# lym01803/FinalProject-LosslessImageCompression

Measured on AMD Instinct MI355X. Metric: encode+decode Mpixels/s (imagenet64, bit-exact round trip), higher is better.
Workload: dtype f32

## Files before the change

finalproject-losslessimagecompression_amd/csrc/conv3_dx3.hip:

```cpp
#include <hip/hip_runtime.h>
#include <stdint.h>

#include <utility>

#include "idf_cdf.h"
#include "idf_codec_internal.h"
#include "wino_common.h"

#pragma clang fp contract(off)

namespace idf {

typedef float d4 __attribute__((ext_vector_type(4)));
typedef _Float16 e4 __attribute__((ext_vector_type(4)));
typedef _Float16 e8 __attribute__((ext_vector_type(8)));
typedef unsigned int v4u __attribute__((ext_vector_type(4)));
typedef __bf16 b8 __attribute__((ext_vector_type(8)));

struct Dx3Args {
  const uint16_t* xs;
  int64_t P;
  int64_t xs_pix, xs_slab, xs_bytes;
  int32_t nslab_xs;
  int32_t C;
  const uint16_t* Wt;
  int32_t nslab, ngroup;
  int32_t N;
  int32_t B, H, Wd;
  int32_t nbx, nby;
  int32_t tiles_x, tiles_y, ntiles, nblk_tiles;
  int32_t ch;
  int32_t seg, segw, nseg;
  int32_t gut, wp, hp;
  int32_t tilew, xskip;
  int32_t nchunk, chunk_slabs;
  float* part;
  uint32_t* ctr;
  const float* b3;
  const float* vtap;
  const float* bfull;
  int32_t ldv;
  int32_t act;
  float slope;
  float* out;
  int64_t ldo;
  float yscale;
  uint32_t* flag;
  const float* hw;
  int32_t ldhw, nh;
  float* hacc;
  int32_t hlast, skip_f32, hmode, hn_mean;
  float* hout;
  int64_t hld_out;
  const float* hbase;
  int64_t hld_base;
  float *hmean, *hlogs, *hscale;
};

#ifndef IDF_DX3_ABLATE
#define IDF_DX3_ABLATE 0
#endif
#ifndef IDF_DX3_DB
#define IDF_DX3_DB 3
#endif
#ifndef IDF_DX3_SB
#define IDF_DX3_SB 1
#endif
// ... 7 lines not shown
#define IDF_DX3_STAG 0
#endif
#ifndef IDF_DX3_STAMPS
#define IDF_DX3_STAMPS 0
#endif
#ifndef IDF_DX3_STAMP_BLOCK
#define IDF_DX3_STAMP_BLOCK 100
#endif
#if IDF_DX3_STAMPS
__device__ unsigned long long g_dx3_stamp[8][40][4];
__device__ unsigned long long g_dx3_phase[8][6];
#define DX3_PHASE(j, v)                                                                      \
  do {                                                                                      \
    if (blockIdx.x == IDF_DX3_STAMP_BLOCK && lane == 0) g_dx3_phase[wave][(j)] = (v);       \
  } while (0)
#define DX3_STAMP(slab, j)                                                                 \
  do {                                                                                    \
    if (blockIdx.x == IDF_DX3_STAMP_BLOCK && (slab) < 40 && lane == 0)                    \
      g_dx3_stamp[wave][(slab)][(j)] = __builtin_amdgcn_s_memtime();                      \
  } while (0)
#else
#define DX3_STAMP(slab, j) do { } while (0)
#define DX3_PHASE(j, v) do { } while (0)
#endif
#ifndef IDF_DX3_TL
#define IDF_DX3_TL 0
#endif
#if IDF_DX3_TL
__device__ unsigned long long g_dx3_tl[4096][8];
#define DX3_TL(j)                                                                          \
  do {                                                                                    \
    if (tid == 0 && blockIdx.x < 4096) g_dx3_tl[blockIdx.x][(j)] = __builtin_amdgcn_s_memrealtime(); \
  } while (0)
#else
#define DX3_TL(j) do { } while (0)
#endif
#ifndef IDF_DX3_KSPLIT
#define IDF_DX3_KSPLIT 4
#endif
#ifndef IDF_DX3_KSPLIT16
#define IDF_DX3_KSPLIT16 1
#endif
#ifndef IDF_DX3_TWO_MIN
#define IDF_DX3_TWO_MIN 512
#endif
#ifndef IDF_DX3_FORCE1
#define IDF_DX3_FORCE1 0
#endif

#ifndef IDF_DX3_PAIRS
#define IDF_DX3_PAIRS 0
#endif
#ifndef IDF_DX3_PRIO
#define IDF_DX3_PRIO 0
#endif
#ifndef IDF_DX3_PRIO_K
#define IDF_DX3_PRIO_K 4
#endif
#ifndef IDF_DX3_MIX
#define IDF_DX3_MIX 0
#endif
#ifndef IDF_DX3_WAVES
#define IDF_DX3_WAVES 8
#endif
constexpr int kDxWaves = IDF_DX3_WAVES;
constexpr int kDxThreads = 64 * kDxWaves;
constexpr uint32_t kDxInvalid = 0xFFFFFFF0u;
constexpr uint32_t kDxOff = 0x80000000u;
// ... 137 lines not shown
  static_assert(HR >= 3, "the A-fragment reads of a phase take its last three steps");
  static_assert(IDF_DX3_DMAS == 0 || IDF_DX3_DMA0 + IDF_DX3_STAG + (L::PPW - 1) * IDF_DX3_DMAS < NS,
                "every DMA piece of a slab is issued within the slab's steps");
  int* last_flag = (int*)(lds + L::FOFF);
  const int tid = threadIdx.x, lane = tid & 63;
  const int wave = __builtin_amdgcn_readfirstlane(tid >> 6);
  const int bid = xcd_contiguous(blockIdx.x, gridDim.x);
  const int per_chunk = g.ngroup * g.nblk_tiles;
  const int chunk = udiv_s(bid, per_chunk);
  const int rem = bid - chunk * per_chunk;
  const int grp = udiv_s(rem, g.nblk_tiles);
  const int tb = rem - grp * g.nblk_tiles;
  const int tw = MIX ? (wave & 3) >> 1 : wave / (kDxWaves / T);
  constexpr int WR_OLD = IDF_DX3_MIX == 2 ? WR - 1 : WR + 1;
  const int r0 = MIX ? 2 * WR * (wave & 1) + ((wave & 4) ? WR_OLD : 0) : WR * (wave % (kDxWaves / T));
  d4 hreg[WRW];
  const int nlayers = ML ? ml->nlayers : 1;
  for (int li = 0; li < nlayers; ++li) {
  int tid_o = tid, lane_o = lane, wave_o = wave, tb_o = tb, tw_o = tw, r0_o = r0, grp_o = grp,
      chunk_o = chunk;
  if constexpr (ML) {
    asm volatile("" : "+v"(tid_o), "+v"(lane_o), "+v"(wave_o), "+v"(tb_o), "+v"(tw_o), "+v"(r0_o),
                 "+v"(grp_o), "+v"(chunk_o));
    wave_o = __builtin_amdgcn_readfirstlane(wave_o);
    tb_o = __builtin_amdgcn_readfirstlane(tb_o);
    tw_o = __builtin_amdgcn_readfirstlane(tw_o);
    r0_o = __builtin_amdgcn_readfirstlane(r0_o);
    grp_o = __builtin_amdgcn_readfirstlane(grp_o);
    chunk_o = __builtin_amdgcn_readfirstlane(chunk_o);
  }
  const int tid = tid_o, lane = lane_o, wave = wave_o, tb = tb_o, tw = tw_o, r0 = r0_o,
            grp = grp_o, chunk = chunk_o;
  const int lz = 0;
  Dx3Layer Ly;
  if constexpr (ML) {
    Ly = ml->layer[li];
  } else {
    Ly = Dx3Layer{g.Wt, g.b3, g.vtap, g.bfull, g.out, g.yscale, g.C, g.nslab, g.nchunk,
                  g.chunk_slabs, g.hlast};
  }
  const int tile = tb * T + tw + lz;

  const int64_t plane_b = g.P * 32;
  const int xs_rec = (int)(g.xs_slab < (int64_t)kDxInvalid ? g.xs_slab : (int64_t)kDxInvalid);
  uint32_t pbase[L::PPW];
  int plo[L::PPW];
  bool pok[L::PPW];
#pragma unroll
  for (int i = 0; i < L::PPW; ++i) {
    const bool hk = i < L::PH;
    const int k = wave + kDxWaves * (hk ? i : i - L::PH);
    pok[i] = k < (hk ? L::HPIECES : L::WPIECES);
    pbase[i] = kDxOff;
    plo[i] = 0;
    if (hk && pok[i]) {
      const int t = k / (L::NPL * PLANE_KIB), pl = (k / PLANE_KIB) % L::NPL, pi = k % PLANE_KIB;
      plo[i] = (t * L::NPL + pl) * L::PLANE + pi * 1024;
      const int slot = 32 * pi + (lane >> 1);
      const int tt = tb * T + t;
      if (tt < g.ntiles) {
        const DxTile dt = dx_tile(g, tt);
        int ix, x, iy, y;
        bool ok;
        if (g.gut) {
          const int cr = slot / PITCH, cc = slot - cr * PITCH;
          const int u = dt.u0 - 1 + cc, uy = dt.u0y - 1 + cr;
          ix = u >= 0 ? udiv_s(u, g.wp) : 0;
          x = u >= 0 ? u - ix * g.wp : -1;
          iy = uy >= 0 ? udiv_s(uy, g.hp) : 0;
          y = uy >= 0 ? uy - iy * g.hp : -1;
          ok = cr < g.ch && cc < g.segw;
        } else {
          const int sk = g.seg ? udiv_s(slot, g.seg) : 0;
          const int rr = slot - sk * g.seg;
          const int cr = rr / PITCH, cc = rr - cr * PITCH;
          ok = sk < g.nseg && cc < g.segw && cr < g.ch;
          ix = dt.ix0 + sk;
          x = (sk ? 0 : dt.xf0) - 1 + cc;
          const int vy = dt.vy0 + cr;
          iy = udiv_s(vy, g.H + 2);
          y = vy - iy * (g.H + 2) - 1;
        }
        const int b = (dt.band * g.nby + iy) * g.nbx + ix;
        ok = ok && x >= 0 && x < g.Wd && ix < g.nbx && y >= 0 && y < g.H && iy < g.nby && b < g.B;
        if (ok)
          pbase[i] = (uint32_t)(pl * plane_b + ((((int64_t)b * g.H + y) * g.Wd + x) * g.xs_pix) + (lane & 1) * 16);
      }
    } else if (!hk && pok[i]) {
      plo[i] = L::WOFF + k * 1024;
      pbase[i] = (uint32_t)(grp * L::WST + k * 1024 + lane * 16);
    }
  }
  DX3_TL(0);
  for (int e = tid; e < NF * 512 / 16; e += kDxThreads) *(d4*)(lds + L::ZOFF + 16 * e) = d4{0.f, 0.f, 0.f, 0.f};
  DX3_PHASE(0, __builtin_amdgcn_s_memtime());
  DX3_PHASE(4, __builtin_amdgcn_s_memrealtime());

  const int j = lane & 15, q = lane >> 4;
  const DxTile dt = dx_tile(g, tile < g.ntiles ? tile : 0);
  const int jx = g.xskip ? 3 * (j >> 1) + (j & 1) : j;
  const int uj = dt.u0 + jx;
  const int pw = g.gut ? g.wp : g.Wd;
  const int ixj = udiv_s(uj, pw);
  const int xj = uj - ixj * pw;
  const int kj = ixj - dt.ix0;
  const int colb = g.gut ? jx : kj * g.seg + (kj ? j - (ixj * g.Wd - dt.u0) : j);
  const int uyw = dt.u0y + r0;
  int iyw = udiv_s(uyw, g.H);
  if (iyw > g.nby - 1) iyw = g.nby - 1;
  const int rowb = g.gut ? r0 : uyw + 2 * iyw - dt.vy0;

  const int slot0 = rowb * PITCH + colb;
  const int tb0 = tw * L::NPL * L::PLANE;
  const int oP = tb0 + (q >> 1) * L::PLANE + slot0 * 32 + (q & 1) * 16;
  const int oF = tb0 + slot0 * 32 + (q & 1) * 16 + (q >> 1) * 32;
  const int oG = tb0 + slot0 * 32 + (q & 1) * 16 + 64 + (q >> 1) * PITCH * 32;
  const int oAH = L::WOFF + j * 32 + (q & 1) * 16;
  constexpr int WLO = BF ? 0 : L::WPART;
  const int oAF = L::WOFF + WLO + j * 32 + (q & 1) * 16 + (q >> 1) * NF * 512;
  const int oAG = L::WOFF + WLO + 2 * NF * 512 + j * 32 + (q & 1) * 16 + (q >> 1) * 3 * NF * 512;
  const int oAO = L::WOFF + WLO + 8 * NF * 512 + j * 32 + (q & 1) * 16;
  const int oAHF = L::WOFF + j * 32 + (q & 1) * 16 + (q >> 1) * NF * 512;
  const int oAHG = L::WOFF + 2 * NF * 512 + j * 32 + (q & 1) * 16 + (q >> 1) * 3 * NF * 512;
  const bool zlane = q < 2;
  const char* zO = lds + L::ZOFF + j * 32 + (q & 1) * 16;

  if constexpr (ML) if (li == 0) {
// ... 3 lines not shown
      const bool lane_ok0 = xj < g.Wd && ixj < g.nbx;
#pragma unroll
      for (int m = 0; m < WRW; ++m) {
        int iy = iyw, y = uyw + m - iyw * g.H;
        if (g.gut) {
          iy = udiv_s(uyw + m, g.hp);
          y = uyw + m - iy * g.hp;
        }
        const int img = (dt.band * g.nby + iy) * g.nbx + ixj;
        const bool ok = lane_ok0 && y < g.H && iy < g.nby && img < g.B;
        if (ok && 4 * q < g.nh) {
          const float* xr = ml->hx + (((int64_t)img * g.H + y) * g.Wd + xj) * ml->hld_x;
          d4 h;
#pragma unroll
          for (int i = 0; i < 4; ++i) h[i] = 4 * q + i < g.nh ? ml->hb[4 * q + i] : 0.0f;
          for (int c = 0; c < ml->hc0; c += 4) {
            const d4 xv = *(const d4*)(xr + c);
#pragma unroll
            for (int i = 0; i < 4; ++i) {
              const int o = 4 * q + i;
              if (o < g.nh) {
                const d4 wv = *(const d4*)(g.hw + (int64_t)o * g.ldhw + c);
#pragma unroll
                for (int k = 0; k < 4; ++k) h[i] = __builtin_fmaf(wv[k], xv[k], h[i]);
              }
            }
          }
          hreg[m] = h;
        }
      }
    }
  }

  const int s0 = ML ? 0 : chunk * Ly.chunk_slabs;
  const int s1 = ML ? Ly.nslab : min(Ly.nslab, s0 + Ly.chunk_slabs);
  const uint32_t wslab = (uint32_t)(g.ngroup * L::WST);
  const int64_t wbytes = (int64_t)Ly.nslab * wslab;
  const __amdgpu_buffer_rsrc_t wr = __builtin_amdgcn_make_buffer_rsrc(
      (void*)Ly.Wt, 0, (int)(wbytes < (int64_t)kDxInvalid ? wbytes : (int64_t)kDxInvalid), 0x00020000);
  auto dma = [&](int s, int st, int i) {
    if (!pok[i]) return;
    const bool halo = i < L::PH;
    if (halo ? (IDF_DX3_ABLATE & 1) : (IDF_DX3_ABLATE & 4)) return;
    const __amdgpu_buffer_rsrc_t xr = __builtin_amdgcn_make_buffer_rsrc(
        (void*)((const char*)g.xs + (int64_t)s * g.xs_slab), 0, xs_rec, 0x00020000);
    const uint32_t off = pbase[i] + (halo ? 0u : (uint32_t)(s * g.ngroup) * (uint32_t)L::WST);
    __builtin_amdgcn_raw_ptr_buffer_load_lds(halo ? xr : wr,
                                             (dx_lds_ptr_t)(lds + st * L::STAGE + plo[i]), 16,
                                             off, 0, 0, 0);
  };

  if (s1 > s0) {
#pragma unroll
    for (int i = 0; i < L::PPW; ++i) dma(s0, 0, i);
  }
  Dx3Tables<NF> tabs;
  DX3_PHASE(1, __builtin_amdgcn_s_memtime());
  DX3_TL(1);


  d4 acc[WRW][NF];
#pragma unroll
  for (int m = 0; m < WRW; ++m)
#pragma unroll
    for (int n = 0; n < NF; ++n) acc[m][n] = d4{0.f, 0.f, 0.f, 0.f};

  auto rd = [](const char* p) { return *(const e8*)p; };
  auto mma = [](const e8& a, const e8& bb, d4& c) {
    if (IDF_DX3_ABLATE & 16) c[0] += (float)(a[0] * bb[0]);
    else if constexpr (BF)
      c = __builtin_amdgcn_mfma_f32_16x16x32_bf16(__builtin_bit_cast(b8, a), __builtin_bit_cast(b8, bb),
                                                   c, 0, 0, 0);
    else c = __builtin_amdgcn_mfma_f32_16x16x32_f16(a, bb, c, 0, 0, 0);
  };
  auto rdB = [&](const char* p) -> e8 {
    if (IDF_DX3_ABLATE & 32) return e8{(_Float16)1, (_Float16)(lane & 7), 0, 0, 0, 0, 0, (_Float16)(p == nullptr)};
    return rd(p);
  };
  auto rdA = [&](const char* p) -> e8 {
    if (IDF_DX3_ABLATE & 64) return e8{(_Float16)2, (_Float16)(lane & 3), 0, 0, 0, 0, 0, (_Float16)(p == nullptr)};
    return rd(p);
  };

  constexpr int DB = IDF_DX3_DB, RB = DB + 1;
  e8 Bq[RB];
  e8 AS[2][3][NF];
  e8 AZ[2][NF];
  auto read_B = [&](const char* st, int t) -> e8 {
    if (t < 3 * HR) return rdB(st + oP + ((t % HR) * PITCH + t / HR) * 32);
    if (t < 4 * HR) return rdB(st + oF + (t - 3 * HR) * PITCH * 32);
    return rdB(st + oG + (t - 4 * HR) * PITCH * 32);
  };
  auto read_A = [&](const char* st, int p, int dy, e8 (&A)[NF]) {
#pragma unroll
    for (int n = 0; n < NF; ++n)
      A[n] = p < 3 ? rdA(st + oAH + ((dy * 3 + p) * NF + n) * 512)
                   : rdA(st + oAF + (3 * dy * NF + n) * 512);
  };
  auto mma_rows = [&](const e8 (&A)[3][NF], const e8& Bv, int h) {
#pragma unroll
    for (int dy = 0; dy < 3; ++dy) {
      const int m = h - dy;
      if (m < 0 || m >= WRW) continue;
#pragma unroll
      for (int n = 0; n < NF; ++n) mma(A[dy][n], Bv, acc[m][n]);
    }
  };

  for (int s = s0; s < s1; ++s) {
    const char* cur = lds + ((s - s0) & 1) * L::STAGE;
    DX3_STAMP(s - s0, 0);
    asm volatile("s_waitcnt vmcnt(0) lgkmcnt(0)" ::: "memory");
    if (!(IDF_DX3_ABLATE & 8)) __builtin_amdgcn_s_barrier();
    DX3_STAMP(s - s0, 1);
    if (s == s0) DX3_TL(2);
    if (s == s0) tabs.load(g, Ly, grp, tid);
    if (s == s0 + 1) tabs.store((float*)(lds + L::BOFF), (float*)(lds + L::HOFF), g, Ly, grp, tid);
    __builtin_amdgcn_sched_barrier(0);
    const bool more = s + 1 < s1;
    const int nst = (s + 1 - s0) & 1;
    auto dma_step = [&](auto tc) {
      constexpr int t = decltype(tc)::value;
      constexpr int ds = IDF_DX3_DMAS > 0 ? IDF_DX3_DMAS : 1;
      auto dma_at = [&](auto dtc) {
        constexpr int dt_ = decltype(dtc)::value;
        if constexpr (IDF_DX3_DMAS == 0 && dt_ == 0) {
          if (more) {
#pragma unroll
            for (int i = 0; i < L::PPW; ++i) dma(s + 1, nst, i);
          }
        } else if constexpr (IDF_DX3_DMAS > 0 && dt_ >= 0 && dt_ % ds == 0 && dt_ / ds < L::PPW) {
          if (more) dma(s + 1, nst, dt_ / ds);
        }
      };
      if (IDF_DX3_STAG == 0 || !(wave & 4)) dma_at(std::integral_constant<int, t - IDF_DX3_DMA0>{});
      else dma_at(std::integral_constant<int, t - IDF_DX3_DMA0 - IDF_DX3_STAG>{});
    };
    if constexpr (BF) {
      auto read_Bf = [&](const char* st, int t) -> e8 {
        if (t < HR) return rdB(st + oF + t * PITCH * 32);
        return rdB(st + oG + (t - HR) * PITCH * 32);
      };
#pragma unroll
      for (int k = 0; k < (DB > 3 ? DB : 3); ++k) {
        if (k < DB) Bq[k] = read_Bf(cur, k);
        if (k < 3) read_A(cur, 3, k, AS[1][k]);
      }
      auto stepb = [&](auto tc) {
// ... 124 lines not shown
      if constexpr (t < 3) read_A(cur, 1, t, AS[1][t]);
      if constexpr (t >= HR && t < HR + 3) read_A(cur, 2, t - HR, AS[0][t - HR]);
      if constexpr (t >= 2 * HR && t < 2 * HR + 3) read_A(cur, 3, t - 2 * HR, AS[1][t - 2 * HR]);
      if constexpr (t == 2 * HR + 3 || t == 2 * HR + 4) {
#pragma unroll
        for (int n = 0; n < NF; ++n) {
          if (t == 2 * HR + 3) AZ[0][n] = rdA(cur + oAG + n * 512);
          else AZ[1][n] = rdA(zlane ? zO + n * 512 : cur + oAO + n * 512);
        }
      }
      if constexpr (t + DB < NS) Bq[(t + DB) % RB] = read_B(cur, t + DB);
      const e8& Bv = Bq[t % RB];
      if constexpr (t < 3 * HR) {
        mma_rows(AS[(t / HR) & 1], Bv, t % HR);
      } else if constexpr (t < 4 * HR) {
        mma_rows(AS[1], Bv, t - 3 * HR);
      } else {
        constexpr int h = t - 4 * HR;
        if constexpr (h < WRW) {
#pragma unroll
          for (int n = 0; n < NF; ++n) mma(AZ[0][n], Bv, acc[h][n]);
        }
        if constexpr (h > 0) {
#pragma unroll
          for (int n = 0; n < NF; ++n) mma(AZ[1][n], Bv, acc[h - 1][n]);
        }
      }
    };
    dx_unroll(step, std::make_integer_sequence<int, NS>{});
    DX3_STAMP(s - s0, 3);
  }
  DX3_PHASE(2, __builtin_amdgcn_s_memtime());
  DX3_TL(3);
  if (s1 - s0 <= 1) {
    if (s1 == s0) tabs.load(g, Ly, grp, tid);
    tabs.store((float*)(lds + L::BOFF), (float*)(lds + L::HOFF), g, Ly, grp, tid);
  }
  if (s1 - s0 <= 2) __syncthreads();

  if constexpr (T == 1 && !ML) if (Ly.nchunk > 1) {
    constexpr int FR = kDxWaves * WR * NF;
    const uint32_t pb = (uint32_t)((tb * g.ngroup + grp) * Ly.nchunk) * (FR * 1024u);
    const int64_t pbytes = (int64_t)g.nblk_tiles * g.ngroup * Ly.nchunk * FR * 1024;
    const __amdgpu_buffer_rsrc_t pr = __builtin_amdgcn_make_buffer_rsrc(
        (void*)g.part, 0, (int)(pbytes < (int64_t)kDxInvalid ? pbytes : (int64_t)kDxInvalid), 0x00020000);
    auto poff = [&](int c, int m, int n) -> uint32_t {
      return pb + (uint32_t)((c * FR + (tw * 16 + r0 + m) * NF + n) * 1024 + lane * 16);
    };
#pragma unroll
    for (int m = 0; m < WRW; ++m)
#pragma unroll
      for (int n = 0; n < NF; ++n)
        __builtin_amdgcn_raw_buffer_store_b128(__builtin_bit_cast(v4u, acc[m][n]), pr, poff(chunk, m, n),
                                               0, 16 );
    asm volatile("s_waitcnt vmcnt(0)" ::: "memory");
    __syncthreads();
    if (tid == 0) {
      const uint32_t old = __hip_atomic_fetch_add(g.ctr + tb * g.ngroup + grp, 1u, __ATOMIC_RELAXED,
                                                  __HIP_MEMORY_SCOPE_AGENT);
      const bool last = old == (uint32_t)(Ly.nchunk - 1);
      if (last)
        __hip_atomic_store(g.ctr + tb * g.ngroup + grp, 0u, __ATOMIC_RELAXED, __HIP_MEMORY_SCOPE_AGENT);
      *last_flag = last;
    }
    __syncthreads();
    DX3_TL(6);
// ... 25 lines not shown

  if (tile >= g.ntiles) return;
  const bool lane_ok = xj < g.Wd && ixj < g.nbx;
  const WAct act(g.act, g.slope);
  const float* btab = (const float*)(lds + L::BOFF);
  const float* htab = (const float*)(lds + L::HOFF);
  const bool fh = g.nh > 0;
  bool out_ok = true;
  const int zr = (Ly.C + g.N + 15) / 16 * 16, zend = zr < 16 * g.nslab_xs ? zr : 16 * g.nslab_xs;
  const bool lastg = grp == g.ngroup - 1;
  char* xsb = (char*)g.xs;
  int r_img[WRW], r_y[WRW];
  int64_t r_pix[WRW];
  bool r_ok[WRW];
#pragma unroll
  for (int m = 0; m < WRW; ++m) {
    int iy = iyw, y = uyw + m - iyw * g.H;
    if (g.gut) {
      iy = udiv_s(uyw + m, g.hp);
      y = uyw + m - iy * g.hp;
    }
    r_img[m] = (dt.band * g.nby + iy) * g.nbx + ixj;
    r_y[m] = y;
    r_ok[m] = lane_ok && y < g.H && iy < g.nby && r_img[m] < g.B;
    r_pix[m] = ((int64_t)r_img[m] * g.H + y) * g.Wd + xj;
  }
  d4 hprev[WRW];
#pragma unroll
  for (int m = 0; m < WRW; ++m) {
    hprev[m] = d4{0.f, 0.f, 0.f, 0.f};
    if constexpr (ML) hprev[m] = hreg[m];
    else if (fh && r_ok[m] && 4 * q < g.nh) hprev[m] = *(const d4*)(g.hacc + r_pix[m] * 16 + 4 * q);
  }
#pragma unroll
  for (int m = 0; m < WRW; ++m) {
    const bool row_ok = r_ok[m];
    if (!row_ok && !fh) continue;
    const int cls = bias_class(r_y[m], xj, g.H, g.Wd);
    const int64_t pix = r_pix[m];
    float* dst = Ly.out + pix * g.ldo;
#pragma unroll
    for (int n = 0; n <= NF; ++n) {
      if (n == NF && !lastg) break;
      const int nl = 16 * n + 4 * q;
      const int n0 = 16 * grp * NF + nl;
      d4 v = d4{0.f, 0.f, 0.f, 0.f};
      if (n < NF && n0 < g.N) {
        const d4 bv = *(const d4*)(btab + cls * (NF * 16) + nl);
#pragma unroll
        for (int k = 0; k < 4; ++k) {
          const float t = acc[m][n][k] * Ly.yscale + bv[k];
          v[k] = act.tanh_ ? wact(t, g.act, g.slope) : act(t);
          if (!BF && row_ok) out_ok = out_ok && fabsf(v[k]) < kDxOutGuard;
        }
        if (row_ok && !g.skip_f32) {
          if (n0 + 4 <= g.N) {
            *(d4*)(dst + n0) = v;
          } else {
#pragma unroll
            for (int k = 0; k < 4; ++k)
              if (n0 + k < g.N) dst[n0 + k] = v[k];
          }
        }
        for (int k = g.N - n0; k < 4; ++k) v[k] = 0.0f;
      }
      if (n < NF) acc[m][n] = v;
      const int c = Ly.C + n0;
      if (row_ok && !(IDF_DX3_ABLATE & 128) && c < zend) {
        if constexpr (BF) {
          typedef __bf16 b4 __attribute__((ext_vector_type(4)));
          *(b4*)(xsb + (int64_t)(c >> 4) * g.xs_slab + pix * g.xs_pix + (c & 15) * 2) =
              __builtin_convertvector(v, b4);
        } else {
          const e4 h = __builtin_convertvector(v, e4);
          const e4 l = __builtin_convertvector(v - __builtin_convertvector(h, d4), e4);
          char* p = xsb + (int64_t)(c >> 4) * 2 * plane_b + pix * 32 + (c & 15) * 2;
          *(e4*)p = h;
          *(e4*)(p + plane_b) = l;
        }
      }
    }
  }
  if (fh) {
    float hp[WRW][16];
#pragma unroll
    for (int m = 0; m < WRW; ++m)
#pragma unroll
      for (int o = 0; o < 16; ++o) hp[m][o] = 0.0f;
#pragma unroll
    for (int n = 0; n < NF; ++n) {
      const int nl = 16 * n + 4 * q;
      if (16 * grp * NF + nl >= g.N) continue;
#pragma unroll
      for (int o = 0; o < 16; ++o) {
        if (o < g.nh) {
          const d4 wv = *(const d4*)(htab + o * (NF * 16) + nl);
#pragma unroll
          for (int m = 0; m < WRW; ++m)
#pragma unroll
            for (int k = 0; k < 4; ++k) hp[m][o] = __builtin_fmaf(wv[k], acc[m][n][k], hp[m][o]);
        }
      }
    }
#pragma unroll
    for (int m = 0; m < WRW; ++m) {
      float r8[8], r4[4];
#pragma unroll
      for (int i = 0; i < 8; ++i) {
        const float mine = q < 2 ? hp[m][i] : hp[m][8 + i];
        const float give = q < 2 ? hp[m][8 + i] : hp[m][i];
        r8[i] = mine + __shfl_xor(give, 32);
      }
#pragma unroll
      for (int i = 0; i < 4; ++i) {
        const float mine = (q & 1) ? r8[4 + i] : r8[i];
// ... 15 lines not shown
          const int64_t hw_ = (int64_t)g.H * g.Wd, rem = (int64_t)r_y[m] * g.Wd + xj;
#pragma unroll
          for (int i = 0; i < 4; ++i) {
            const int o = 4 * q + i;
            if (o >= g.nh) break;
            const float vv = hv[i];
            if (g.hmode == IDF_EPI_COUPLE_ADD || g.hmode == IDF_EPI_COUPLE_SUB) {
              const float r = __builtin_rintf(vv * 256.0f) / 256.0f;
              const float bsv = g.hbase[pix * g.hld_base + o];
              g.hout[pix * g.hld_out + o] = g.hmode == IDF_EPI_COUPLE_ADD ? bsv + r : bsv - r;
            } else if (g.hmode == IDF_EPI_PRIOR) {
              if (o < g.hn_mean) {
                g.hmean[((int64_t)b_img * g.hn_mean + o) * hw_ + rem] = vv;
              } else {
                const int64_t oi = ((int64_t)b_img * g.hn_mean + (o - g.hn_mean)) * hw_ + rem;
                g.hlogs[oi] = vv;
                g.hscale[oi] = expf_glibc(vv);
              }
            } else {
              g.hout[pix * g.hld_out + o] = vv;
            }
          }
        }
      }
    }
  }
  if (!out_ok && g.flag) atomicOr(g.flag, 1u);
  DX3_TL(5);
  DX3_PHASE(3, __builtin_amdgcn_s_memtime());
  DX3_PHASE(5, __builtin_amdgcn_s_memrealtime());
  if constexpr (ML) {
    asm volatile("s_waitcnt vmcnt(0) lgkmcnt(0)" ::: "memory");
    __builtin_amdgcn_s_barrier();
  }
  }
}

template <int NF, int WR, int PITCH, int PLANE_KIB, bool BF>
__global__ void __launch_bounds__(kDxThreads, 1) conv3_dx3_kernel(Dx3Args g) {
  __shared__ __attribute__((aligned(16))) char lds[Dx3Lds<NF, WR, PITCH, PLANE_KIB, BF>::BYTES];
  if constexpr (IDF_DX3_MIX && !BF && WR * kDxWaves == 32 && WR >= 2) {
    constexpr int D = IDF_DX3_MIX == 2 ? -1 : 1;
    if (threadIdx.x < 256) dx3_block<NF, WR, PITCH, PLANE_KIB, BF, false, WR + D>(g, nullptr, lds);
    else dx3_block<NF, WR, PITCH, PLANE_KIB, BF, false, WR - D>(g, nullptr, lds);
  } else {
    dx3_block<NF, WR, PITCH, PLANE_KIB, BF, false>(g, nullptr, lds);
  }
}

template <int NF, int PITCH, int PLANE_KIB, bool BF>
__global__ void __launch_bounds__(kDxThreads, 1) conv3_dx3_block_kernel(Dx3Args g, Dx3MLArgs ml) {
  __shared__ __attribute__((aligned(16))) char lds[Dx3Lds<NF, 16 / kDxWaves, PITCH, PLANE_KIB, BF>::BYTES];
  dx3_block<NF, 16 / kDxWaves, PITCH, PLANE_KIB, BF, true>(g, &ml, lds);
}

__device__ __forceinline__ void dx3_head_init_pixel(int64_t p, int32_t C0, const float* __restrict__ x,
                                                    int64_t ld_x, const float* __restrict__ w,
                                                    int32_t ldw, const float* __restrict__ bias,
                                                    int32_t nh, float* __restrict__ acc) {
  float h[16];
#pragma unroll
  for (int o = 0; o < 16; ++o) h[o] = o < nh ? bias[o] : 0.0f;
  const float* xr = x + p * ld_x;
  for (int c = 0; c < C0; c += 4) {
    const d4 xv = *(const d4*)(xr + c);
#pragma unroll
// ... 101 lines not shown
      p.nby = 1;
      p.ch = 18;
    }
    int sg = p.ch * p.pitch;
    while ((sg - W) % 8) ++sg;
    p.seg = sg;
    p.ok = (p.nseg * sg * 32 + 1023) / 1024 <= p.plane_kib;
  }
  if (!p.ok) {
    p.gut = 1; p.wp = W + 1; p.hp = H + 1;
    p.nbx = 16 / dx3_gcd(p.wp, 16);
    while (p.nbx > 1 && p.nbx * p.wp > 128) p.nbx /= 2;
    p.nby = 16 / dx3_gcd(p.hp, 16);
    while (p.nby > 1 && p.nby * p.hp > 128) p.nby /= 2;
    p.pitch = 18; p.ch = 18; p.segw = 18; p.nseg = 1; p.seg = 0; p.plane_kib = 11;
    p.ok = 1;
    if (W == 2 && !bf) {
      p.xskip = 1; p.tilew = 24; p.pitch = 25; p.segw = 25; p.plane_kib = 15;
    }
  }
  p.split = (H * W <= 64 && p.nbx * p.nby <= 4) ? IDF_DX3_KSPLIT
            : (H == 16 && W == 16) ? IDF_DX3_KSPLIT16 : 1;
  return p;
}

}

using namespace idf;

#if IDF_DX3_TL
extern "C" int idf_dx3_timeline(unsigned long long* host) {
  return hipMemcpyFromSymbol(host, HIP_SYMBOL(g_dx3_tl), sizeof(g_dx3_tl)) == hipSuccess ? 0 : 2;
}
#endif

#if IDF_DX3_STAMPS
extern "C" int idf_dx3_stamps(unsigned long long* host) {
  if (hipMemcpyFromSymbol(host, HIP_SYMBOL(g_dx3_stamp), sizeof(g_dx3_stamp)) != hipSuccess) return 2;
  return hipMemcpyFromSymbol(host + 8 * 40 * 4, HIP_SYMBOL(g_dx3_phase), sizeof(g_dx3_phase)) == hipSuccess ? 0 : 2;
}
#endif

namespace {

int dx3_tiles_x(const Dx3Plan& p, int W) {
  return (p.nbx * (p.gut ? p.wp : W) + p.tilew - 1) / p.tilew;
}
int dx3_tiles_y(const Dx3Plan& p, int H) { return (p.nby * (p.gut ? p.hp : H) + 15) / 16; }

struct Dx3Launch {
  Dx3Plan pl;
  int64_t ntiles;
  int T, nblk_tiles, nslab, nchunk, chunk_slabs;
  int64_t ctr_bytes, part_bytes;
};

Dx3Launch dx3_launch_shape(int B, int H, int W, int C, int N, bool bf = false) {
  Dx3Launch s = {};
  s.pl = dx3_plan(H, W, N, bf);
  if (!s.pl.ok || B < 1) return s;
  const int64_t nbands = (B + s.pl.nbx * s.pl.nby - 1) / (s.pl.nbx * s.pl.nby);
  const int tiles_x = dx3_tiles_x(s.pl, W), tiles_y = dx3_tiles_y(s.pl, H);
  s.ntiles = nbands * tiles_x * tiles_y;
  s.nslab = (C + 15) / 16;
  s.chunk_slabs = s.nslab > 0 ? (s.nslab + s.pl.split - 1) / s.pl.split : 1;
  s.nchunk = s.nslab > 0 ? (s.nslab + s.chunk_slabs - 1) / s.chunk_slabs : 1;
// ... 78 lines not shown
#ifndef IDF_HEAD_INIT_EXTERNAL
__global__ void __launch_bounds__(256) dx3_head_init_kernel(int64_t P, int32_t C0,
                                                            const float* __restrict__ x,
                                                            int64_t ld_x, const float* __restrict__ w,
                                                            int32_t ldw, const float* __restrict__ bias,
                                                            int32_t nh, float* __restrict__ acc) {
  const int64_t p = (int64_t)blockIdx.x * blockDim.x + threadIdx.x;
  if (p >= P) return;
  dx3_head_init_pixel(p, C0, x, ld_x, w, ldw, bias, nh, acc);
}

extern "C" int idf_dx3_head_init(void* stream, int64_t P, int32_t C0, const float* x, int64_t ld_x,
                                 const float* w, int32_t ldw, const float* bias, int32_t n_head,
                                 float* acc) {
  if (P <= 0) return P < 0 ? IDF_ERR_ARG : IDF_OK;
  if (!x || !w || !bias || !acc || n_head < 1 || n_head > 16 || C0 < 0 || C0 > 64 || (C0 & 3) ||
      (ld_x & 3) || (uintptr_t)x % 16 || (uintptr_t)acc % 16 || ldw < C0 || (ldw & 3) ||
      (uintptr_t)w % 16)
    return IDF_ERR_ARG;
  hipLaunchKernelGGL(dx3_head_init_kernel, dim3((unsigned)((P + 255) / 256)), dim3(256), 0,
                     (hipStream_t)stream, P, C0, x, ld_x, w, ldw, bias, n_head, acc);
  return idf_last_error();
}
#endif

static bool dxb_plan_ok(const Dx3Plan& p) {
  return p.ok && p.nf <= 3 && p.ngroup == 1 && (p.pitch == 18 || p.pitch == 10);
}

extern "C" int idf_conv3x3_dxb_supported(int32_t H, int32_t W, int32_t N) {
  return dxb_plan_ok(dx3_plan(H, W, N, true)) ? 1 : 0;
}

static int dx3_args(Dx3Args& g, Dx3Launch& sh, bool ml, bool bf, int32_t B, int32_t H, int32_t W,
                    int32_t C, uint16_t* xs, int64_t xs_pix, int64_t xs_slab, int64_t xs_bytes,
                    int32_t nslab_xs, const uint16_t* w, int32_t nft, float yscale, const float* b3,
                    const float* vtap, int32_t ldv, const float* bfull, int32_t N, float* out,
                    int64_t ld_out, int32_t act, float slope, uint32_t* d_flag, void* d_workspace,
                    int64_t workspace_bytes, const IdfDx3Head* head) {
  if (C <= 0 || (C & 3) || !w || !xs || !out || !b3) return IDF_ERR_ARG;
  sh = dx3_launch_shape(B, H, W, C, N, bf);
  if (!sh.pl.ok || (bf && !dxb_plan_ok(sh.pl))) return IDF_ERR_UNSUPPORTED;
  if (ml) {
    sh.T = 1;
    sh.nblk_tiles = (int)sh.ntiles;
  }
  if (nft != sh.pl.ngroup * sh.pl.nf) return IDF_ERR_ARG;
  if (vtap && (!bfull || ldv < N)) return IDF_ERR_ARG;
  if ((uintptr_t)out % 16 || ld_out % 4) return IDF_ERR_ARG;
  if ((C + 15) / 16 > nslab_xs) return IDF_ERR_ARG;
  const int64_t P = (int64_t)B * H * W;
  if (xs_slab >= (int64_t)kDxOff) return IDF_ERR_UNSUPPORTED;
  const int64_t nblk = (int64_t)sh.nblk_tiles * sh.pl.ngroup * (ml ? 1 : sh.nchunk);
  if (sh.ntiles >= (1 << 20) || nblk >= (1 << 20)) return IDF_ERR_UNSUPPORTED;
  g = {};
  if (sh.nchunk > 1 && !ml) {
    if (nblk * (int64_t)(kDxWaves * (16 / kDxWaves) * sh.pl.nf) * 1024 >= (int64_t)kDxInvalid)
      return IDF_ERR_UNSUPPORTED;
    const int64_t cb = idf_conv3x3_dx3_counter_bytes(B, H, W, N);
    if (!d_workspace || (uintptr_t)d_workspace % 256 || workspace_bytes < cb + sh.part_bytes)
      return IDF_ERR_WORKSPACE;
    g.ctr = (uint32_t*)d_workspace;
    g.part = (float*)((char*)d_workspace + cb);
  }
  g.xs = xs; g.P = P; g.nslab_xs = nslab_xs; g.C = C;
  g.xs_pix = xs_pix; g.xs_slab = xs_slab; g.xs_bytes = xs_bytes;
  g.Wt = w; g.nslab = sh.nslab; g.ngroup = sh.pl.ngroup; g.N = N;
  g.B = B; g.H = H; g.Wd = W;
  g.nbx = sh.pl.nbx; g.nby = sh.pl.nby;
  g.tiles_x = dx3_tiles_x(sh.pl, W);
  g.tiles_y = dx3_tiles_y(sh.pl, H);
  g.ntiles = (int32_t)sh.ntiles;
  g.nblk_tiles = sh.nblk_tiles;
  g.ch = sh.pl.ch; g.seg = sh.pl.seg; g.segw = sh.pl.segw; g.nseg = sh.pl.nseg;
  g.gut = sh.pl.gut; g.wp = sh.pl.wp; g.hp = sh.pl.hp;
  g.tilew = sh.pl.tilew; g.xskip = sh.pl.xskip;
  g.nchunk = sh.nchunk; g.chunk_slabs = sh.chunk_slabs;
  g.b3 = b3; g.vtap = vtap; g.bfull = bfull; g.ldv = ldv; g.act = act; g.slope = slope;
  g.out = out; g.ldo = ld_out; g.yscale = yscale; g.flag = d_flag;
  if (head && head->n_head > 0) {
    if (head->n_head > 16 || sh.pl.ngroup != 1 || !head->w || (!head->acc && !ml) ||
        head->ldw < C + N || (uintptr_t)head->acc % 16)
      return IDF_ERR_ARG;
    const IdfHeadOut& o = head->out;
    if (head->last || ml) {
      if (o.mode == IDF_EPI_PRIOR ? (!o.mean || !o.logscale || !o.scale || o.n_mean < 0 ||
                                     2 * o.n_mean != head->n_head)
                                  : (!o.out || ((o.mode == IDF_EPI_COUPLE_ADD ||
                                                 o.mode == IDF_EPI_COUPLE_SUB) && !o.base)))
        return IDF_ERR_ARG;
    }
    g.hw = head->w; g.ldhw = head->ldw; g.nh = head->n_head; g.hacc = head->acc;
    g.hlast = head->last; g.skip_f32 = head->skip_f32; g.hmode = o.mode; g.hn_mean = o.n_mean;
    g.hout = o.out; g.hld_out = o.ld_out; g.hbase = o.base; g.hld_base = o.ld_base;
    g.hmean = o.mean; g.hlogs = o.logscale; g.hscale = o.scale;
  } else if (head && head->skip_f32) {
    g.skip_f32 = 1;
  }
  return IDF_OK;
}

static int dx3_run(void* stream, bool bf, int32_t B, int32_t H, int32_t W, int32_t C, uint16_t* xs,
                   int64_t xs_pix, int64_t xs_slab, int64_t xs_bytes, int32_t nslab_xs,
                   const uint16_t* w, int32_t nft, float yscale, const float* b3,
                   const float* vtap, int32_t ldv, const float* bfull, int32_t N, float* out,
                   int64_t ld_out, int32_t act, float slope, uint32_t* d_flag, void* d_workspace,
                   int64_t workspace_bytes, const IdfDx3Head* head) {
  if (B <= 0 || H <= 0 || W <= 0 || N <= 0) return IDF_OK;
  Dx3Args g;
// ... 207 lines not shown
```

Measured before the change: 21.39.

## Issue weight DMA early, add fast halo addressing, specialize tanh epilogue

Moves the weight-slab buffer descriptor and first-stage weight DMA ahead of the halo address computation, so weight loads are in flight while halo addresses are being computed. Adds a fast halo addressing path for non-gutter, single-segment plans with pitch 18. It uses per-tile origins made wave-uniform instead of per-lane divisions. It also zeroes the LDS zero region only on the first layer of multi-layer launches and splits the output epilogue into compile-time tanh and non-tanh variants with the bias loads hoisted. Risks are a correctness mismatch in the fast addressing for edge tiles and higher register pressure.

```diff
diff --git a/finalproject-losslessimagecompression_amd/csrc/conv3_dx3.hip b/finalproject-losslessimagecompression_amd/csrc/conv3_dx3.hip
--- a/finalproject-losslessimagecompression_amd/csrc/conv3_dx3.hip
+++ b/finalproject-losslessimagecompression_amd/csrc/conv3_dx3.hip
@@ -1,6 +1,9 @@
 #include <hip/hip_runtime.h>
 #include <stdint.h>
-
+#include <stdlib.h>
+#include <string.h>
+
+#include <type_traits>
 #include <utility>
 
 #include "idf_cdf.h"
@@ -33,6 +36,7 @@
   int32_t seg, segw, nseg;
   int32_t gut, wp, hp;
   int32_t tilew, xskip;
+  int32_t fastplan;
   int32_t nchunk, chunk_slabs;
   float* part;
   uint32_t* ctr;
@@ -106,8 +110,15 @@
   do {                                                                                    \
     if (tid == 0 && blockIdx.x < 4096) g_dx3_tl[blockIdx.x][(j)] = __builtin_amdgcn_s_memrealtime(); \
   } while (0)
+__device__ unsigned long long g_dx3_tlml[1024][16][4];
+#define DX3_TLML(li, j)                                                                    \
+  do {                                                                                    \
+    if (ML && tid == 0 && blockIdx.x < 1024 && (li) < 16)                                 \
+      g_dx3_tlml[blockIdx.x][(li)][(j)] = __builtin_amdgcn_s_memrealtime();               \
+  } while (0)
 #else
 #define DX3_TL(j) do { } while (0)
+#define DX3_TLML(li, j) do { } while (0)
 #endif
 #ifndef IDF_DX3_KSPLIT
 #define IDF_DX3_KSPLIT 4
@@ -311,6 +322,7 @@
   const int tid = tid_o, lane = lane_o, wave = wave_o, tb = tb_o, tw = tw_o, r0 = r0_o,
             grp = grp_o, chunk = chunk_o;
   const int lz = 0;
+  DX3_TLML(li, 0);
   Dx3Layer Ly;
   if constexpr (ML) {
     Ly = ml->layer[li];
@@ -325,19 +337,72 @@
   uint32_t pbase[L::PPW];
   int plo[L::PPW];
   bool pok[L::PPW];
-#pragma unroll
-  for (int i = 0; i < L::PPW; ++i) {
-    const bool hk = i < L::PH;
-    const int k = wave + kDxWaves * (hk ? i : i - L::PH);
-    pok[i] = k < (hk ? L::HPIECES : L::WPIECES);
+  const int s0 = ML ? 0 : chunk * Ly.chunk_slabs;
+  const int s1 = ML ? Ly.nslab : min(Ly.nslab, s0 + Ly.chunk_slabs);
+  const uint32_t wslab = (uint32_t)(g.ngroup * L::WST);
+  const int64_t wbytes = (int64_t)Ly.nslab * wslab;
+  const __amdgpu_buffer_rsrc_t wr = __builtin_amdgcn_make_buffer_rsrc(
+      (void*)Ly.Wt, 0, (int)(wbytes < (int64_t)kDxInvalid ? wbytes : (int64_t)kDxInvalid), 0x00020000);
+  auto dma = [&](int s, int st, int i) {
+    if (!pok[i]) return;
+    const bool halo = i < L::PH;
+    if (halo ? (IDF_DX3_ABLATE & 1) : (IDF_DX3_ABLATE & 4)) return;
+    const __amdgpu_buffer_rsrc_t xr = __builtin_amdgcn_make_buffer_rsrc(
+        (void*)((const char*)g.xs + (int64_t)s * g.xs_slab), 0, xs_rec, 0x00020000);
+    const uint32_t off = pbase[i] + (halo ? 0u : (uint32_t)(s * g.ngroup) * (uint32_t)L::WST);
+    __builtin_amdgcn_raw_ptr_buffer_load_lds(halo ? xr : wr,
+                                             (dx_lds_ptr_t)(lds + st * L::STAGE + plo[i]), 16,
+                                             off, 0, 0, 0);
+  };
+#pragma unroll
+  for (int i = L::PH; i < L::PPW; ++i) {
+    const int k = wave + kDxWaves * (i - L::PH);
+    pok[i] = k < L::WPIECES;
+    plo[i] = pok[i] ? L::WOFF + k * 1024 : 0;
+    pbase[i] = pok[i] ? (uint32_t)(grp * L::WST + k * 1024 + lane * 16) : kDxOff;
+    if (s1 > s0) dma(s0, 0, i);
+  }
+  uint32_t forg[T] = {};
+  int fu0[T] = {}, fy0[T] = {};
+  if constexpr (PITCH == 18) if (g.fastplan) {
+#pragma unroll
+    for (int t = 0; t < T; ++t) {
+      const int tt = tb * T + t;
+      const DxTile dtt = dx_tile(g, tt < g.ntiles ? tt : 0);
+      const bool tok = tt < g.ntiles && dtt.band < g.B;
+      fu0[t] = __builtin_amdgcn_readfirstlane(dtt.u0 - 1);
+      fy0[t] = __builtin_amdgcn_readfirstlane(tok ? dtt.u0y - 1 : INT32_MIN / 2);
+      forg[t] = __builtin_amdgcn_readfirstlane(
+          ((uint32_t)dtt.band * (uint32_t)g.H + (uint32_t)(dtt.u0y - 1)) * (uint32_t)g.Wd + (uint32_t)(dtt.u0 - 1));
+    }
+  }
+#pragma unroll
+  for (int i = 0; i < L::PH; ++i) {
+    const int k = wave + kDxWaves * i;
+    pok[i] = k < L::HPIECES;
     pbase[i] = kDxOff;
     plo[i] = 0;
-    if (hk && pok[i]) {
+    if (pok[i]) {
       const int t = k / (L::NPL * PLANE_KIB), pl = (k / PLANE_KIB) % L::NPL, pi = k % PLANE_KIB;
       plo[i] = (t * L::NPL + pl) * L::PLANE + pi * 1024;
       const int slot = 32 * pi + (lane >> 1);
       const int tt = tb * T + t;
-      if (tt < g.ntiles) {
+      bool fast = false;
+      if constexpr (PITCH == 18) fast = g.fastplan != 0;
+      if (fast) {
+        const int cr = slot / PITCH, cc = slot - cr * PITCH;
+        int u0m = fu0[0], y0m = fy0[0];
+        uint32_t org = forg[0];
+#pragma unroll
+        for (int u = 1; u < T; ++u)
+          if (t == u) { u0m = fu0[u]; y0m = fy0[u]; org = forg[u]; }
+        const bool ok = (uint32_t)(u0m + cc) < (uint32_t)g.Wd && (uint32_t)(y0m + cr) < (uint32_t)g.H &&
+                        cr < PITCH;
+        if (ok)
+          pbase[i] = (uint32_t)pl * (uint32_t)plane_b +
+                     (org + (uint32_t)cr * (uint32_t)g.Wd + (uint32_t)cc) * (uint32_t)g.xs_pix +
+                     (uint32_t)((lane & 1) * 16);
+      } else if (tt < g.ntiles) {
         const DxTile dt = dx_tile(g, tt);
         int ix, x, iy, y;
         bool ok;
@@ -365,13 +430,12 @@
         if (ok)
           pbase[i] = (uint32_t)(pl * plane_b + ((((int64_t)b * g.H + y) * g.Wd + x) * g.xs_pix) + (lane & 1) * 16);
       }
-    } else if (!hk && pok[i]) {
-      plo[i] = L::WOFF + k * 1024;
-      pbase[i] = (uint32_t)(grp * L::WST + k * 1024 + lane * 16);
-    }
+    }
+    if (s1 > s0) dma(s0, 0, i);
   }
   DX3_TL(0);
-  for (int e = tid; e < NF * 512 / 16; e += kDxThreads) *(d4*)(lds + L::ZOFF + 16 * e) = d4{0.f, 0.f, 0.f, 0.f};
+  if (!ML || li == 0)
+    for (int e = tid; e < NF * 512 / 16; e += kDxThreads) *(d4*)(lds + L::ZOFF + 16 * e) = d4{0.f, 0.f, 0.f, 0.f};
   DX3_PHASE(0, __builtin_amdgcn_s_memtime());
   DX3_PHASE(4, __builtin_amdgcn_s_memrealtime());
 
@@ -441,28 +505,6 @@
     }
   }
 
-  const int s0 = ML ? 0 : chunk * Ly.chunk_slabs;
-  const int s1 = ML ? Ly.nslab : min(Ly.nslab, s0 + Ly.chunk_slabs);
-  const uint32_t wslab = (uint32_t)(g.ngroup * L::WST);
-  const int64_t wbytes = (int64_t)Ly.nslab * wslab;
-  const __amdgpu_buffer_rsrc_t wr = __builtin_amdgcn_make_buffer_rsrc(
-      (void*)Ly.Wt, 0, (int)(wbytes < (int64_t)kDxInvalid ? wbytes : (int64_t)kDxInvalid), 0x00020000);
-  auto dma = [&](int s, int st, int i) {
-    if (!pok[i]) return;
-    const bool halo = i < L::PH;
-    if (halo ? (IDF_DX3_ABLATE & 1) : (IDF_DX3_ABLATE & 4)) return;
-    const __amdgpu_buffer_rsrc_t xr = __builtin_amdgcn_make_buffer_rsrc(
-        (void*)((const char*)g.xs + (int64_t)s * g.xs_slab), 0, xs_rec, 0x00020000);
-    const uint32_t off = pbase[i] + (halo ? 0u : (uint32_t)(s * g.ngroup) * (uint32_t)L::WST);
-    __builtin_amdgcn_raw_ptr_buffer_load_lds(halo ? xr : wr,
-                                             (dx_lds_ptr_t)(lds + st * L::STAGE + plo[i]), 16,
-                                             off, 0, 0, 0);
-  };
-
-  if (s1 > s0) {
-#pragma unroll
-    for (int i = 0; i < L::PPW; ++i) dma(s0, 0, i);
-  }
   Dx3Tables<NF> tabs;
   DX3_PHASE(1, __builtin_amdgcn_s_memtime());
   DX3_TL(1);
@@ -523,6 +565,7 @@
     if (!(IDF_DX3_ABLATE & 8)) __builtin_amdgcn_s_barrier();
     DX3_STAMP(s - s0, 1);
     if (s == s0) DX3_TL(2);
+    if (s == s0) DX3_TLML(li, 1);
     if (s == s0) tabs.load(g, Ly, grp, tid);
     if (s == s0 + 1) tabs.store((float*)(lds + L::BOFF), (float*)(lds + L::HOFF), g, Ly, grp, tid);
     __builtin_amdgcn_sched_barrier(0);
@@ -713,6 +756,7 @@
   }
   DX3_PHASE(2, __builtin_amdgcn_s_memtime());
   DX3_TL(3);
+  DX3_TLML(li, 2);
   if (s1 - s0 <= 1) {
     if (s1 == s0) tabs.load(g, Ly, grp, tid);
     tabs.store((float*)(lds + L::BOFF), (float*)(lds + L::HOFF), g, Ly, grp, tid);
@@ -804,55 +848,66 @@
     if constexpr (ML) hprev[m] = hreg[m];
     else if (fh && r_ok[m] && 4 * q < g.nh) hprev[m] = *(const d4*)(g.hacc + r_pix[m] * 16 + 4 * q);
   }
-#pragma unroll
-  for (int m = 0; m < WRW; ++m) {
-    const bool row_ok = r_ok[m];
-    if (!row_ok && !fh) continue;
-    const int cls = bias_class(r_y[m], xj, g.H, g.Wd);
-    const int64_t pix = r_pix[m];
-    float* dst = Ly.out + pix * g.ldo;
-#pragma unroll
-    for (int n = 0; n <= NF; ++n) {
-      if (n == NF && !lastg) break;
-      const int nl = 16 * n + 4 * q;
-      const int n0 = 16 * grp * NF + nl;
-      d4 v = d4{0.f, 0.f, 0.f, 0.f};
-      if (n < NF && n0 < g.N) {
-        const d4 bv = *(const d4*)(btab + cls * (NF * 16) + nl);
-#pragma unroll
-        for (int k = 0; k < 4; ++k) {
-          const float t = acc[m][n][k] * Ly.yscale + bv[k];
-          v[k] = act.tanh_ ? wact(t, g.act, g.slope) : act(t);
-          if (!BF && row_ok) out_ok = out_ok && fabsf(v[k]) < kDxOutGuard;
-        }
-        if (row_ok && !g.skip_f32) {
-          if (n0 + 4 <= g.N) {
-            *(d4*)(dst + n0) = v;
+  auto outputs = [&](auto tanh_c) {
+    constexpr bool TANH = decltype(tanh_c)::value;
+#pragma unroll
+    for (int m = 0; m < WRW; ++m) {
+      const bool row_ok = r_ok[m];
+      if (!row_ok && !fh) continue;
+      const int cls = bias_class(r_y[m], xj, g.H, g.Wd);
+      const int64_t pix = r_pix[m];
+      float* dst = Ly.out + pix * g.ldo;
+      d4 bv[NF];
+#pragma unroll
+      for (int n = 0; n < NF; ++n) bv[n] = *(const d4*)(btab + cls * (NF * 16) + 16 * n + 4 * q);
+#pragma unroll
+      for (int n = 0; n <= NF; ++n) {
+        if (n == NF && !lastg) break;
+        const int nl = 16 * n + 4 * q;
+        const int n0 = 16 * grp * NF + nl;
+        d4 v = d4{0.f, 0.f, 0.f, 0.f};
+        if (n < NF) {
+          const bool live = n0 < g.N;
+#pragma unroll
+          for (int k = 0; k < 4; ++k) {
+            const float t = acc[m][n][k] * Ly.yscale + bv[n][k];
+            if constexpr (TANH) v[k] = wact(t, g.act, g.slope);
+            else v[k] = act(t);
+            if (!BF) out_ok = out_ok && (!(live && row_ok) || fabsf(v[k]) < kDxOutGuard);
+          }
+          if (live && row_ok && !g.skip_f32) {
+            if (n0 + 4 <= g.N) {
+              *(d4*)(dst + n0) = v;
+            } else {
+#pragma unroll
+              for (int k = 0; k < 4; ++k)
+                if (n0 + k < g.N) dst[n0 + k] = v[k];
+            }
+          }
+#pragma unroll
+          for (int k = 0; k < 4; ++k) v[k] = n0 + k < g.N ? v[k] : 0.0f;
+          acc[m][n] = v;
+        }
+        const int c = Ly.C + n0;
+        if (row_ok && !(IDF_DX3_ABLATE & 128) && c < zend) {
+          if constexpr (BF) {
+            typedef __bf16 b4 __attribute__((ext_vector_type(4)));
+            *(b4*)(xsb + (int64_t)(c >> 4) * g.xs_slab + pix * g.xs_pix + (c & 15) * 2) =
+                __builtin_convertvector(v, b4);
           } else {
-#pragma unroll
-            for (int k = 0; k < 4; ++k)
-              if (n0 + k < g.N) dst[n0 + k] = v[k];
+            const e4 h = __builtin_convertvector(v, e4);
+            const e4 l = __builtin_convertvector(v - __builtin_convertvector(h, d4), e4);
+            char* p = xsb + (int64_t)(c >> 4) * 2 * plane_b + pix * 32 + (c & 15) * 2;
+            *(e4*)p = h;
+            *(e4*)(p + plane_b) = l;
           }
         }
-        for (int k = g.N - n0; k < 4; ++k) v[k] = 0.0f;
-      }
-      if (n < NF) acc[m][n] = v;
-      const int c = Ly.C + n0;
-      if (row_ok && !(IDF_DX3_ABLATE & 128) && c < zend) {
-        if constexpr (BF) {
-          typedef __bf16 b4 __attribute__((ext_vector_type(4)));
-          *(b4*)(xsb + (int64_t)(c >> 4) * g.xs_slab + pix * g.xs_pix + (c & 15) * 2) =
-              __builtin_convertvector(v, b4);
-        } else {
-          const e4 h = __builtin_convertvector(v, e4);
-          const e4 l = __builtin_convertvector(v - __builtin_convertvector(h, d4), e4);
-          char* p = xsb + (int64_t)(c >> 4) * 2 * plane_b + pix * 32 + (c & 15) * 2;
-          *(e4*)p = h;
-          *(e4*)(p + plane_b) = l;
-        }
-      }
-    }
-  }
+      }
+    }
+  };
+  if (act.tanh_) outputs(std::true_type{});
+  else outputs(std::false_type{});
+  DX3_TL(7);
   if (fh) {
     float hp[WRW][16];
 #pragma unroll
@@ -934,6 +989,7 @@
   if constexpr (ML) {
     asm volatile("s_waitcnt vmcnt(0) lgkmcnt(0)" ::: "memory");
     __builtin_amdgcn_s_barrier();
+    DX3_TLML(li, 3);
   }
   }
 }
@@ -1101,6 +1157,9 @@
 extern "C" int idf_dx3_timeline(unsigned long long* host) {
   return hipMemcpyFromSymbol(host, HIP_SYMBOL(g_dx3_tl), sizeof(g_dx3_tl)) == hipSuccess ? 0 : 2;
 }
+extern "C" int idf_dx3_timeline_ml(unsigned long long* host) {
+  return hipMemcpyFromSymbol(host, HIP_SYMBOL(g_dx3_tlml), sizeof(g_dx3_tlml)) == hipSuccess ? 0 : 2;
+}
 #endif
 
 #if IDF_DX3_STAMPS
@@ -1245,6 +1304,11 @@
   return dxb_plan_ok(dx3_plan(H, W, N, true)) ? 1 : 0;
 }
 
+static bool dx3_plan_generic() {
+  const char* e = getenv("IDF_DX3_PLAN");
+  return e && !strcmp(e, "generic");
+}
+
 static int dx3_args(Dx3Args& g, Dx3Launch& sh, bool ml, bool bf, int32_t B, int32_t H, int32_t W,
                     int32_t C, uint16_t* xs, int64_t xs_pix, int64_t xs_slab, int64_t xs_bytes,
                     int32_t nslab_xs, const uint16_t* w, int32_t nft, float yscale, const float* b3,
@@ -1288,6 +1352,7 @@
   g.ch = sh.pl.ch; g.seg = sh.pl.seg; g.segw = sh.pl.segw; g.nseg = sh.pl.nseg;
   g.gut = sh.pl.gut; g.wp = sh.pl.wp; g.hp = sh.pl.hp;
   g.tilew = sh.pl.tilew; g.xskip = sh.pl.xskip;
+  g.fastplan = !sh.pl.gut && sh.pl.nseg == 1 && sh.pl.pitch == 18 && !dx3_plan_generic();
   g.nchunk = sh.nchunk; g.chunk_slabs = sh.chunk_slabs;
   g.b3 = b3; g.vtap = vtap; g.bfull = bfull; g.ldv = ldv; g.act = act; g.slope = slope;
   g.out = out; g.ldo = ld_out; g.yscale = yscale; g.flag = d_flag;
```

Result: faster. 21.87 (median of 6 runs) (+2.2%).
